# maffos/Diffusion-Modelling-for-inverse-problems

Hardware: NVIDIA B200
Metric: score-net evals/sec (posterior sampler) (higher is better)
Workload: dtype bf16

## Files before the change

### diffusion-modelling-for-inverse-problems_b200/csrc/dmip_rng.cuh

```cuda
#pragma once
#include <stdint.h>

namespace dmip {

constexpr uint32_t kPhiloxStepInit = 0xFFFFFFFFu;
constexpr uint32_t kStreamState = 0;
constexpr uint32_t kStreamObs = 1;

__device__ __forceinline__ void philox4x32_10(uint32_t c0, uint32_t c1, uint32_t c2, uint32_t c3, uint32_t k0,
                                              uint32_t k1, uint32_t (&out)[4]) {
#pragma unroll
  for (int r = 0; r < 10; ++r) {
    const uint32_t hi0 = __umulhi(0xD2511F53u, c0), lo0 = 0xD2511F53u * c0;
    const uint32_t hi1 = __umulhi(0xCD9E8D57u, c2), lo1 = 0xCD9E8D57u * c2;
    c0 = hi1 ^ c1 ^ k0;
    c1 = lo1;
    c2 = hi0 ^ c3 ^ k1;
    c3 = lo0;
    k0 += 0x9E3779B9u;
    k1 += 0xBB67AE85u;
  }
  out[0] = c0; out[1] = c1; out[2] = c2; out[3] = c3;
}

__device__ __forceinline__ float u01(uint32_t r) { return (static_cast<float>(r >> 8) + 0.5f) * (1.0f / 16777216.0f); }

__device__ __forceinline__ void philox_normal4(uint64_t gidx, uint32_t step, uint32_t stream, uint32_t quad,
                                               uint64_t seed, float (&z)[4]) {
  uint32_t r[4];
  philox4x32_10(static_cast<uint32_t>(gidx), static_cast<uint32_t>(gidx >> 32), step, (stream << 16) | quad,
                static_cast<uint32_t>(seed), static_cast<uint32_t>(seed >> 32), r);
#pragma unroll
  for (int j = 0; j < 2; ++j) {
    const float u1 = u01(r[2 * j]), u2 = u01(r[2 * j + 1]);
    float R;
    asm("sqrt.approx.ftz.f32 %0, %1;" : "=f"(R) : "f"(fmaxf(-2.0f * __logf(u1), 0.0f)));
    float s, c;
    __sincosf(6.283185307179586f * u2, &s, &c);
    z[2 * j] = R * c;
    z[2 * j + 1] = R * s;
  }
}

}
```

### diffusion-modelling-for-inverse-problems_b200/csrc/dmip_tc.cu

```cuda
#include <stdlib.h>

#include "dmip_common.h"
#include "dmip_ptx.cuh"
#include "dmip_rng.cuh"
#include "dmip_sde.cuh"

namespace dmip {

namespace {

constexpr int kTileM = 128;
constexpr int kStageBytes = 16384;
constexpr int kNumSlots = 6;
constexpr int kNumPairs = kNumSlots / 2;
constexpr int kPairBytes = 2 * kStageBytes;
constexpr int kHBytes = 131072;
constexpr int kThreads = 640;
constexpr int kRegsSmall = 32;
constexpr int kRegsRow = 112;
constexpr int kNumRowWarps = 16;
constexpr int kRowThreads = 512;
constexpr int kProducerWarp = 16;
constexpr int kMmaWarp = 17;
#ifndef DMIP_CLUSTER
#define DMIP_CLUSTER 2
#endif
constexpr int kCluster = DMIP_CLUSTER;
constexpr uint32_t kTmemCols = 512;
constexpr uint32_t kTmemH = 0;
constexpr uint32_t kTmemAcc = 256;
constexpr uint32_t kTmemL0 = kTmemH + 192;
#ifndef DMIP_L2_TAIL_TMEM
#define DMIP_L2_TAIL_TMEM 1
#endif
constexpr bool kL2TailTmem = DMIP_L2_TAIL_TMEM != 0;

constexpr int kOffH = 0;
constexpr int kOffB = kOffH + kHBytes;
constexpr int kOffB0 = kOffB + kNumSlots * kStageBytes;
constexpr int kOffB3 = kOffB0 + 2048;
constexpr int kOffBar = kOffB3 + 512;
constexpr int kNumBars = 2 * kNumPairs + 2 + 2 + 1 + 1 + 1 + 4 + 1;
constexpr int kOffTmem = kOffBar + kNumBars * 8;
constexpr int kSmemBytes = kOffTmem + 16;

enum { kModeSampler = 0, kModeForward = 1 };

struct TcNetDev {
  const uint8_t* stages;
  const float* b0;
  const float* b1;
  const float* b2;
  const float* b3;
  const float* w0c;
  int kb0, ksteps0, dv, split, l0_f16, outpad, n_const, n_stages;
  int l0_tmem;
};

struct TcParams {
  int mode, variant, n_nets;
  TcNetDev net[2];
  int xdim, ydim, n_obs, tiles_per_obs, S;
  long long n_per_obs, n_tiles;
  float T, bmin, bmax, mean, std, delta, sqrt_delta;
  int sde_kind, n_corr;
  float snr;
  const float* y;
  float* out;
  int rng_mode;
  unsigned long long seed, gidx_base;
  const float* x0;
  const float* noise;
  const float* ynoise;
  const float* fx;
  const float* fcond;
  const float* ft;
  int fx_dim, fcond_dim, out_dim;
  int dbg;
  int cluster;
  unsigned long long* tl;
  int tl_cap;
};

struct Bars {
  uint64_t* full;
  uint64_t* empty;
  uint64_t* acc_full;
  uint64_t* acc_empty;
  uint64_t* out_full;
  uint64_t* out_empty;
  uint64_t* sh_free;
  uint64_t* hready;
  uint64_t* a0_ready;
};

__device__ __forceinline__ int keep(int v) { return __shfl_sync(0xffffffffu, v, 0); }
__device__ __forceinline__ long long keep(long long v) {
  const unsigned lo = __shfl_sync(0xffffffffu, static_cast<unsigned>(v), 0);
  const unsigned hi = __shfl_sync(0xffffffffu, static_cast<unsigned>(static_cast<unsigned long long>(v) >> 32), 0);
  return static_cast<long long>((static_cast<unsigned long long>(hi) << 32) | lo);
}
template <class T>
__device__ __forceinline__ const T* keep(const T* p) {
  return reinterpret_cast<const T*>(keep(static_cast<long long>(reinterpret_cast<uintptr_t>(p))));
}

__device__ __forceinline__ uint32_t pin_here(uint32_t v) {
  asm volatile("" : "+r"(v) :: "memory");
  return v;
}

template <int kRegs>
__device__ __forceinline__ void reg_dealloc() { asm volatile("setmaxnreg.dec.sync.aligned.u32 %0;" ::"n"(kRegs)); }
template <int kRegs>
__device__ __forceinline__ void reg_alloc() { asm volatile("setmaxnreg.inc.sync.aligned.u32 %0;" ::"n"(kRegs)); }

__device__ __forceinline__ void st_shared_v4(void* p, uint32_t a, uint32_t b, uint32_t c, uint32_t d) {
  asm volatile("st.shared.v4.b32 [%0], {%1, %2, %3, %4};" ::"r"(smem_u32(p)), "r"(a), "r"(b), "r"(c), "r"(d) : "memory");
}

#ifndef DMIP_EPI
#define DMIP_EPI 1
#endif
template <bool kDoubleTanh>
__device__ __forceinline__ void tanh_pack16(const uint32_t (&v)[16], const float* __restrict__ bias, uint32_t (&pk)[8]) {
#pragma unroll
  for (int q = 0; q < 4; ++q) {
    const float4 bq = kDoubleTanh ? *reinterpret_cast<const float4*>(bias + q * 4)
                                  : __ldg(reinterpret_cast<const float4*>(bias + q * 4));
#ifndef DMIP_H_F16
    float a[4];
#pragma unroll
    for (int e = 0; e < 4; ++e) {
      const float bb = e == 0 ? bq.x : e == 1 ? bq.y : e == 2 ? bq.z : bq.w;
      float t = tanh_fast(__uint_as_float(v[q * 4 + e]) + bb);
      if (kDoubleTanh) t = tanh_unit_poly(t);
      a[e] = t;
    }
    pk[q * 2] = pack_bf16x2(a[0], a[1]);
    pk[q * 2 + 1] = pack_bf16x2(a[2], a[3]);
#else
#if DMIP_EPI == 0
    uint32_t t01 = tanh_f16x2(pack_f16x2(__uint_as_float(v[q * 4 + 0]) + bq.x, __uint_as_float(v[q * 4 + 1]) + bq.y));
    uint32_t t23 = tanh_f16x2(pack_f16x2(__uint_as_float(v[q * 4 + 2]) + bq.z, __uint_as_float(v[q * 4 + 3]) + bq.w));
    if (kDoubleTanh) {
      t01 = tanh_unit_poly_f16x2(t01);
      t23 = tanh_unit_poly_f16x2(t23);
    }
#elif DMIP_EPI == 1
    float a[4];
#pragma unroll
    for (int e = 0; e < 4; ++e) {
      const float bb = e == 0 ? bq.x : e == 1 ? bq.y : e == 2 ? bq.z : bq.w;
      float t = tanh_fast(__uint_as_float(v[q * 4 + e]) + bb);
      if (kDoubleTanh) t = tanh_unit_poly(t);
      a[e] = t;
    }
    uint32_t t01 = pack_f16x2(a[0], a[1]), t23 = pack_f16x2(a[2], a[3]);
#else
    float a[4];
#pragma unroll
    for (int e = 0; e < 4; ++e) {
      const float bb = e == 0 ? bq.x : e == 1 ? bq.y : e == 2 ? bq.z : bq.w;
      a[e] = tanh_fast(__uint_as_float(v[q * 4 + e]) + bb);
    }
    uint32_t t01 = pack_f16x2(a[0], a[1]), t23 = pack_f16x2(a[2], a[3]);
    if (kDoubleTanh) {
      t01 = tanh_unit_poly_f16x2(t01);
      t23 = tanh_unit_poly_f16x2(t23);
    }
#endif
    pk[q * 2] = t01;
    pk[q * 2 + 1] = t23;
#endif
  }
}

struct NoExtra {
  __device__ __forceinline__ void operator()() const {}
};

template <bool kDoubleTanh, bool kToTmem, class Extra = NoExtra>
__device__ __forceinline__ void epi_hidden(uint32_t lane_taddr, uint32_t acc_col, int cgp, int row, int chunk, int lane,
                                           const float* __restrict__ bias, uint8_t* sH, uint64_t* acc_empty,
                                           uint64_t* hready, Extra extra = NoExtra()) {
  const int n0 = chunk * 128 + cgp * 32;
  uint32_t v[16], pk[8];
  tmem_ld16(lane_taddr + acc_col + cgp * 32, v);
  tc_wait_ld();
  extra();
  tanh_pack16<kDoubleTanh>(v, bias + n0, pk);
  uint8_t* rowp = sH + (chunk * 2 + (cgp >> 1)) * kStageBytes + (row >> 3) * 1024 + (row & 7) * 128;
  const int c0 = (cgp & 1) * 4;
  if (kToTmem) {
    tmem_st8(lane_taddr + kTmemH + static_cast<uint32_t>(n0 >> 1), pk);
  } else {
    st_shared_v4(rowp + (((c0 + 0) ^ (row & 7)) << 4), pk[0], pk[1], pk[2], pk[3]);
    st_shared_v4(rowp + (((c0 + 1) ^ (row & 7)) << 4), pk[4], pk[5], pk[6], pk[7]);
  }
  tmem_ld16(lane_taddr + acc_col + cgp * 32 + 16, v);
  tc_wait_ld();
  tc_fence_before();
  __syncwarp();
  if (lane == 0) mbar_arrive(acc_empty);
  tanh_pack16<kDoubleTanh>(v, bias + n0 + 16, pk);
  if (kToTmem) {
    tmem_st8(lane_taddr + kTmemH + static_cast<uint32_t>(n0 >> 1) + 8, pk);
    tc_wait_st();
    tc_fence_before();
  } else {
    st_shared_v4(rowp + (((c0 + 2) ^ (row & 7)) << 4), pk[0], pk[1], pk[2], pk[3]);
    st_shared_v4(rowp + (((c0 + 3) ^ (row & 7)) << 4), pk[4], pk[5], pk[6], pk[7]);
    fence_proxy_async_smem();
  }
  __syncwarp();
  if (lane == 0) mbar_arrive(hready);
}

__device__ __forceinline__ void a0_store(uint8_t* sH, int row, int k, float v) {
  const uint32_t off = sw128_offset(static_cast<uint32_t>(row), static_cast<uint32_t>(k), kStageBytes);
  const unsigned short h = static_cast<unsigned short>(pack_bf16x2(v, 0.f) & 0xFFFFu);
  *reinterpret_cast<unsigned short*>(sH + off) = h;
}
__device__ __forceinline__ float f16_clamp(float v) { return fminf(fmaxf(v, -65504.f), 65504.f); }
__device__ __forceinline__ void a0_store_f16(uint8_t* sH, int row, int k, float v) {
  const uint32_t off = sw128_offset(static_cast<uint32_t>(row), static_cast<uint32_t>(k), kStageBytes);
  *reinterpret_cast<unsigned short*>(sH + off) = static_cast<unsigned short>(pack_f16x2(f16_clamp(v), 0.f) & 0xFFFFu);
}
__device__ __forceinline__ void a0_put(uint8_t* sH, int row, int idx, int dvp, int split, float v) {
  if (split == 4) { a0_store_f16(sH, row, idx, v); return; }
  const float hi = bf16_round(v);
  a0_store(sH, row, idx, hi);
  if (split >= 2) a0_store(sH, row, dvp + idx, v - hi);
  if (split >= 3) a0_store(sH, row, 2 * dvp + idx, hi);
}
__device__ __forceinline__ void a0_put8(uint8_t* sH, int row, int idx0, int dvp, int split, const float* v) {
  uint8_t* rowp0 = sH + (row >> 3) * 1024 + (row & 7) * 128;
  if (split == 4) {
    st_shared_v4(rowp0 + (idx0 >> 6) * kStageBytes + ((((idx0 & 63) >> 3) ^ (row & 7)) << 4),
                 pack_f16x2(f16_clamp(v[0]), f16_clamp(v[1])), pack_f16x2(f16_clamp(v[2]), f16_clamp(v[3])),
                 pack_f16x2(f16_clamp(v[4]), f16_clamp(v[5])), pack_f16x2(f16_clamp(v[6]), f16_clamp(v[7])));
    return;
  }
  float hi[8];
#pragma unroll
  for (int e = 0; e < 8; ++e) hi[e] = bf16_round(v[e]);
  const uint32_t h0 = pack_bf16x2(hi[0], hi[1]), h1 = pack_bf16x2(hi[2], hi[3]), h2 = pack_bf16x2(hi[4], hi[5]),
                 h3 = pack_bf16x2(hi[6], hi[7]);
  uint8_t* rowp = sH + (row >> 3) * 1024 + (row & 7) * 128;
  auto chunk_ptr = [&](int k) { return rowp + (k >> 6) * kStageBytes + ((((k & 63) >> 3) ^ (row & 7)) << 4); };
  st_shared_v4(chunk_ptr(idx0), h0, h1, h2, h3);
  if (split >= 2)
    st_shared_v4(chunk_ptr(dvp + idx0), pack_bf16x2(v[0] - hi[0], v[1] - hi[1]), pack_bf16x2(v[2] - hi[2], v[3] - hi[3]),
                 pack_bf16x2(v[4] - hi[4], v[5] - hi[5]), pack_bf16x2(v[6] - hi[6], v[7] - hi[7]));
  if (split >= 3) st_shared_v4(chunk_ptr(2 * dvp + idx0), h0, h1, h2, h3);
}

struct TlRole {
  unsigned long long* p;
  unsigned int n, cap;
  bool minimal;
};
__device__ __forceinline__ TlRole tl_role(const TcParams& P, int dbg, int role, bool on) {
  TlRole r;
  r.p = nullptr;
  r.n = 0;
  r.cap = 0;
  r.minimal = (dbg & 64) != 0;
  if (P.tl != nullptr && blockIdx.x == 0 && on) {
    const int seg = P.tl_cap / 4;
    r.p = P.tl + static_cast<size_t>(role) * seg;
    r.cap = static_cast<unsigned int>(seg - 1);
  }
  return r;
}
__device__ __forceinline__ void tl_mark_impl(TlRole& r, uint32_t code) {
  if (r.p != nullptr && r.n < r.cap && (!r.minimal || code == 0xD00u || (code & 0xF00u) == 0x100u || code == 0xE00u)) {
    r.p[1 + r.n] = (static_cast<unsigned long long>(clock64()) << 16) | code;
    ++r.n;
  }
}
__device__ __forceinline__ void tl_finish_impl(const TlRole& r) {
  if (r.p != nullptr) r.p[0] = r.n;
}
#ifdef DMIP_DEBUG
#define tl_mark(r, code) tl_mark_impl(r, code)
#define tl_finish(r) tl_finish_impl(r)
#define job_mark(r, code) ((void)0)
#elif defined(DMIP_JOBMARKS)
#define tl_mark(r, code) ((void)0)
#define tl_finish(r) tl_finish_impl(r)
#define job_mark(r, code) tl_mark_impl(r, code)
#else
#define tl_mark(r, code) ((void)0)
#define tl_finish(r) ((void)0)
#define job_mark(r, code) ((void)0)
#endif

template <int NP, int VAR>
__global__ void __launch_bounds__(kThreads, 1) k_tc_mlp(const __grid_constant__ TcParams P) {
  constexpr int kOwn = (NP + 3) / 4;
  constexpr bool cdiffe = (VAR == DMIP_CDIFFE);
  constexpr bool dps = (VAR == DMIP_DPS);
  extern __shared__ __align__(1024) uint8_t smem[];
  if ((smem_u32(smem) & 1023u) != 0u) __trap();
  uint8_t* sH = smem + kOffH;
  uint8_t* sB = smem + kOffB;
  float* sB0 = reinterpret_cast<float*>(smem + kOffB0);
  float* sB3 = reinterpret_cast<float*>(smem + kOffB3);
  uint64_t* bars = reinterpret_cast<uint64_t*>(smem + kOffBar);
  uint32_t* tmem_holder = reinterpret_cast<uint32_t*>(smem + kOffTmem);
  Bars B;
  B.full = bars;
  B.empty = bars + kNumPairs;
  B.acc_full = bars + 2 * kNumPairs;
  B.acc_empty = B.acc_full + 2;
  B.out_full = B.acc_empty + 2;
  B.out_empty = B.out_full + 1;
  B.sh_free = B.out_empty + 1;
  B.hready = B.sh_free + 1;
  B.a0_ready = B.hready + 4;

  const int warp = __shfl_sync(0xffffffffu, threadIdx.x >> 5, 0);
  const int lane = threadIdx.x & 31;

  if (warp == kProducerWarp && lane == 0) {
    for (int i = 0; i < kNumPairs; ++i) {
      mbar_init(&B.full[i], 1);
      mbar_init(&B.empty[i], static_cast<uint32_t>(kCluster));
    }
    for (int i = 0; i < 2; ++i) {
      mbar_init(&B.acc_full[i], 1);
      mbar_init(&B.acc_empty[i], kNumRowWarps);
    }
    mbar_init(B.out_full, 1);
    mbar_init(B.out_empty, kNumRowWarps);
    mbar_init(B.sh_free, 1);
    for (int i = 0; i < 4; ++i) mbar_init(&B.hready[i], kNumRowWarps);
    mbar_init(B.a0_ready, kNumRowWarps);
    fence_barrier_init();
  }
  if (warp == kMmaWarp) tmem_alloc<kTmemCols>(tmem_holder);
  for (int i = threadIdx.x; i < kHBytes / 16; i += kThreads) reinterpret_cast<uint4*>(sH)[i] = make_uint4(0, 0, 0, 0);
  for (int i = threadIdx.x; i < 128; i += kThreads) {
    if (dps) sB3[i] = i < 16 ? P.net[i >> 3].b3[i & 7] : 0.f;
    else sB3[i] = P.net[0].b3[i];
  }
  fence_proxy_async_smem();
  tc_fence_before();
  __syncthreads();
  tc_fence_after();
  const uint32_t tmem_base = __shfl_sync(0xffffffffu, *tmem_holder, 0);

  constexpr int C = kCluster;
#ifdef DMIP_DEBUG
  const int dbg = P.dbg & static_cast<int>(*reinterpret_cast<volatile uint32_t*>(tmem_holder) == 0xFFFFFFFFu ? 0u : 0xFFFFFFFFu);
#else
#ifndef DMIP_EXP
#define DMIP_EXP 0
#endif
  constexpr int dbg = DMIP_EXP;
#endif
  const int n_tiles = keep(static_cast<int>(P.n_tiles));
  const uint32_t crank = C > 1 ? cluster_ctarank() : 0u;
  const uint16_t cmask = static_cast<uint16_t>((1u << C) - 1u);
  if (C > 1) cluster_sync_all();
  const int tile_first = static_cast<int>(blockIdx.x / C) * C;
  const int tile_stride = keep(static_cast<int>(gridDim.x));

  const int n_pass = keep(P.n_nets);
  const int S = keep(P.S);
  const int n_steps = keep((P.mode == kModeSampler) ? S * (1 + P.n_corr) : 1);
  constexpr int n_ring = kNumPairs;

  if (warp >= kNumRowWarps) {
    reg_dealloc<kRegsSmall>();
    if (warp == kProducerWarp) {
      int s = 0;
      uint32_t ph = 0;
      TlRole tl = tl_role(P, dbg, 0, lane == 0);
      constexpr uint32_t part = kPairBytes / C;
      for (int tb = tile_first; tb < n_tiles; tb += tile_stride) {
        for (int step = 0; step < n_steps; ++step) {
          for (int p = 0; p < n_pass; ++p) {
            const uint8_t* src = keep(P.net[p].stages);
            const int npairs = keep(P.net[p].n_stages >> 1);
            for (int pr = 0; pr < npairs; ++pr) {
              mbar_wait(&B.empty[s], ph ^ 1u, 0x100 + s);
              tl_mark(tl, 0x600u | (pr & 0xFF));
              const uint8_t* g = src + static_cast<size_t>(pr) * kPairBytes;
              if (elect_one()) {
                if (dbg & 1) {
                  mbar_arrive(&B.full[s]);
                } else {
                  mbar_arrive_expect_tx(&B.full[s], kPairBytes);
                  if (C == 1)
                    bulk_g2s(sB + s * kPairBytes, g, kPairBytes, &B.full[s]);
                  else
                    bulk_g2s_multicast(sB + s * kPairBytes + crank * part, g + crank * part, part, &B.full[s], cmask);
                }
              }
              __syncwarp();
              if (++s == n_ring) { s = 0; ph ^= 1u; }
            }
          }
        }
      }
      tl_finish(tl);
    } else if (warp == kMmaWarp) {
      int s = 0;
      uint32_t ph = 0;
      uint32_t job = 0;
      uint32_t hr_par = 0;
      uint32_t a0_par = 0;
      uint32_t ch0 = 0, ch1 = 0, n_out = 0;
      uint32_t lastkind = 0;
      uint32_t blk = 0;
      TlRole tl = tl_role(P, dbg, 1, lane == 0);
      const uint32_t a_base = (smem_u32(sH) & 0x3FFFFu) >> 4;
      const uint32_t b_base = (smem_u32(sB) & 0x3FFFFu) >> 4;
      const uint64_t desc_hi = umma_smem_desc_sw128(0) & 0xFFFFFFFF00000000ull;
      constexpr uint32_t kBlk16 = kStageBytes >> 4, kPair16 = kPairBytes >> 4;

      auto acquire_acc = [&](int buf, bool is_out, int jl) {
        const uint32_t lk = (lastkind >> (2 * buf)) & 3u;
        tl_mark(tl, 0xB00u | jl);
        if (lk == 1u) mbar_wait(&B.acc_empty[buf], ((buf ? ch1 : ch0) - 1u) & 1u, 0x300 + buf);
        else if (lk == 2u) mbar_wait(B.out_empty, (n_out - 1u) & 1u, 0x310 + buf);
        tl_mark(tl, 0x100u | jl);
        job_mark(tl, 0x100u | jl);
        if (is_out) ++n_out; else { if (buf) ++ch1; else ++ch0; }
        lastkind = (lastkind & ~(3u << (2 * buf))) | ((is_out ? 2u : 1u) << (2 * buf));
      };

      for (int tb = tile_first; tb < n_tiles; tb += tile_stride) {
        for (int step = 0; step < n_steps; ++step) {
          for (int p = 0; p < n_pass; ++p) {
            const int net_kb0 = keep(P.net[p].kb0), net_ksteps0 = keep(P.net[p].ksteps0);
            const uint32_t idesc_out = umma_idesc_bf16(128, static_cast<uint32_t>(keep(P.net[p].outpad)));
            constexpr uint32_t idesc_hid = umma_idesc_bf16(128, 128);
            const uint32_t idesc_l0 = keep(P.net[p].l0_f16) ? umma_idesc_f16(128, 128) : idesc_hid;
            const bool net_l0_tmem = keep(P.net[p].l0_tmem) != 0;
            tl_mark(tl, 0xD00u);
            job_mark(tl, 0xD00u);
            mbar_wait(B.a0_ready, a0_par, 0x200);
            tl_mark(tl, 0xE00u);
            a0_par ^= 1u;
            int jl = 0;
            blk = 0;
#pragma unroll 1
            for (int c = 0; c < 4; ++c, ++job, ++jl) {
              const int buf = job & 1;
              acquire_acc(buf, false, jl);
              const uint32_t d_tmem = tmem_base + kTmemAcc + buf * 128;
#pragma unroll 1
              for (int kb = 0; kb < net_kb0; ++kb, ++blk) {
                const uint32_t half = blk & 1u;
                if (half == 0u) mbar_wait(&B.full[s], ph, 0x500 + s);
                tc_fence_after();
                const int nk = (kb == net_kb0 - 1) ? (net_ksteps0 - 4 * (net_kb0 - 1)) : 4;
                const uint32_t b_lo = b_base + s * kPair16 + half * kBlk16;
                const uint32_t a_lo = a_base + kb * kBlk16;
                if (elect_one()) {
                  if (!(dbg & 2)) {
                    if (net_l0_tmem) {
                      const uint32_t a_tm = tmem_base + kTmemL0 + kb * 32;
#pragma unroll
                      for (int kk = 0; kk < 4; ++kk)
                        if (kk < nk) umma_ts(d_tmem, a_tm + kk * 8, desc_hi | (b_lo + kk * 2), idesc_l0, (kb | kk) != 0 ? 1u : 0u);
                    } else {
#pragma unroll
                      for (int kk = 0; kk < 4; ++kk)
                        if (kk < nk)
                          umma_ss(d_tmem, desc_hi | (a_lo + kk * 2), desc_hi | (b_lo + kk * 2), idesc_l0, (kb | kk) != 0 ? 1u : 0u);
                    }
                  }
                  if (half == 1u) tc_commit_multicast(&B.empty[s], cmask);
                  if (kb == net_kb0 - 1) tc_commit(&B.acc_full[buf]);
                }
                __syncwarp();
                if (half == 1u) { if (++s == n_ring) { s = 0; ph ^= 1u; } }
              }
              tl_mark(tl, 0x200u | jl);
              job_mark(tl, 0x200u | jl);
            }
#pragma unroll 1
            for (int l = 1; l < 4; ++l) {
              const int n_chunks = (l == 3) ? 1 : 4;
#ifndef DMIP_H_F16
              const uint32_t idesc = (l == 3) ? idesc_out : idesc_hid;
#else
              const uint32_t idesc = ((l == 3) ? idesc_out : idesc_hid) & ~((7u << 7) | (7u << 10));
#endif
#pragma unroll 1
              for (int c = 0; c < n_chunks; ++c, ++job, ++jl) {
                const int buf = job & 1;
                acquire_acc(buf, l == 3, jl);
                const uint32_t d_tmem = tmem_base + kTmemAcc + buf * 128;
#pragma unroll 1
                for (int pr = 0; pr < 4; ++pr) {
                  if (c == 0) {
                    mbar_wait(&B.hready[pr], (hr_par >> pr) & 1u, 0x400 + pr);
                    hr_par ^= 1u << pr;
                  }
                  mbar_wait(&B.full[s], ph, 0x500 + s);
                  tc_fence_after();
                  const uint32_t b_lo = b_base + s * kPair16;
                  if (elect_one()) {
                    if (!(dbg & 2)) {
                      if (l == 2 && !(kL2TailTmem && pr == 3)) {
                        const uint32_t a_lo = a_base + pr * kPair16;
#pragma unroll
                        for (int j = 0; j < 8; ++j)
                          umma_ss(d_tmem, desc_hi | (a_lo + (j >> 2) * kBlk16 + (j & 3) * 2),
                                  desc_hi | (b_lo + (j >> 2) * kBlk16 + (j & 3) * 2), idesc, (pr | j) != 0 ? 1u : 0u);
                      } else {
                        const uint32_t a_tm = tmem_base + kTmemH + pr * 64;
#pragma unroll
                        for (int j = 0; j < 8; ++j)
                          umma_ts(d_tmem, a_tm + j * 8, desc_hi | (b_lo + (j >> 2) * kBlk16 + (j & 3) * 2), idesc,
                                  (pr | j) != 0 ? 1u : 0u);
                      }
                    }
                    tc_commit_multicast(&B.empty[s], cmask);
                    if (pr == 3) {
                      if (l == 3) tc_commit(B.out_full);
                      else tc_commit(&B.acc_full[buf]);
                      if (l == 2 && c == 3) tc_commit(B.sh_free);
                    }
                  }
                  __syncwarp();
                  if (++s == n_ring) { s = 0; ph ^= 1u; }
                }
                tl_mark(tl, 0x200u | jl);
                job_mark(tl, 0x200u | jl);
              }
            }
          }
        }
      }
      tl_finish(tl);
    }
  } else {
    reg_alloc<kRegsRow>();
    const int quarter = warp & 3;
    const int cgp = warp >> 2;
    const int row = quarter * 32 + lane;
    const int et = threadIdx.x;
    const uint32_t lane_taddr = tmem_base + (static_cast<uint32_t>(quarter * 32) << 16);
    if (P.net[0].l0_tmem && cgp == 0) {
      const uint32_t z[16] = {0, 0, 0, 0, 0, 0, 0, 0, 0, 0, 0, 0, 0, 0, 0, 0};
#pragma unroll
      for (int c0 = 0; c0 < 64; c0 += 16) tmem_st16(lane_taddr + kTmemL0 + c0, z);
      tc_wait_st();
    }
    asm volatile("bar.sync 2, 512;" ::: "memory");
    TlRole tl = tl_role(P, dbg, warp == 0 ? 2 : 3, lane == 0 && (warp == 0 || warp == 12));
    uint32_t job = 0;
    uint32_t npass = 0;
    uint32_t cf0 = 0, cf1 = 0;
    const SdeSched sch = {P.sde_kind, S, P.n_corr, P.T, P.bmin, P.bmax, P.snr, P.delta, P.sqrt_delta};
    const TcNetDev& net_last = P.net[n_pass - 1];
    const int dvp = (net_last.dv + 7) & ~7;
    const int split = P.net[0].l0_f16 ? 4 : P.net[0].split;
    const bool l0_tmem = P.net[0].l0_tmem != 0;
    const bool sampler = (P.mode == kModeSampler);
    const int xdim = P.xdim;
    const int np = sampler ? (xdim + 7) >> 3 : 0;
    const int pbase = np >> 2, prem = np & 3;
    const int n_own = pbase + (cgp < prem ? 1 : 0);
    const int piece_lo = cgp * pbase + (cgp < prem ? cgp : prem);
    float xs[kOwn * 8];
    float yt[cdiffe ? 8 : 1];
    float myU[2], myWt[2];
#pragma unroll
    for (int j = 0; j < kOwn * 8; ++j) xs[j] = 0.f;
#pragma unroll
    for (int j = 0; j < (cdiffe ? 8 : 1); ++j) yt[j] = 0.f;
    myU[0] = myU[1] = myWt[0] = myWt[1] = 0.f;

    for (int tb = tile_first; tb < n_tiles; tb += tile_stride) {
      const bool tile_ok = tb + static_cast<int>(crank) < n_tiles;
      const int tile = tile_ok ? tb + static_cast<int>(crank) : n_tiles - 1;
      const int obs = static_cast<int>(tile / P.tiles_per_obs);
      const long long prow = static_cast<long long>(tile % P.tiles_per_obs) * kTileM + row;
      const bool valid = tile_ok && prow < P.n_per_obs;
      const long long grow = static_cast<long long>(obs) * P.n_per_obs + prow;
      const unsigned long long gidx = P.gidx_base + static_cast<unsigned long long>(grow);

      auto diffuse_y = [&](int stp) {
        if (!cdiffe) return;
        float g2u, alpha, var;
        sde_terms<true>(sch, sde_substep_tau(sch, stp), g2u, alpha, var);
        const float sd = sqrtf(var);
#pragma unroll
        for (int h = 0; h < 2; ++h) {
          const int q = cgp + 4 * h;
          if (q * 4 < P.ydim) {
            float z[4] = {0.f, 0.f, 0.f, 0.f};
            if (P.rng_mode == DMIP_RNG_PHILOX) philox_normal4(gidx, pin_here(static_cast<uint32_t>(stp)), kStreamObs, q, P.seed, z);
#pragma unroll
            for (int e = 0; e < 4; ++e) {
              const int jj = q * 4 + e;
              float v = 0.f;
              if (valid && jj < P.ydim) {
                const float eta = P.rng_mode == DMIP_RNG_PHILOX
                                      ? z[e]
                                      : P.ynoise[(static_cast<long long>(stp) * (static_cast<long long>(P.n_obs) * P.n_per_obs) + grow) * P.ydim + jj];
                v = fmaf(sd, eta, alpha * P.y[obs * P.ydim + jj]);
              }
              yt[cdiffe ? h * 4 + e : 0] = v;
            }
          }
        }
      };
      auto put_yt = [&]() {
        if (!cdiffe) return;
#pragma unroll
        for (int h = 0; h < 2; ++h)
#pragma unroll
          for (int e = 0; e < 4; ++e) {
            const int jj = (cgp + 4 * h) * 4 + e;
            if (jj < P.ydim) a0_put(sH, row, xdim + jj, dvp, split, yt[cdiffe ? h * 4 + e : 0]);
          }
      };
      auto put_x = [&]() {
#pragma unroll
        for (int i = 0; i < kOwn; ++i) {
          if (i < n_own) {
            const int pc = piece_lo + i;
            if (l0_tmem) {
              const float* v = &xs[i * 8];
              tmem_st4(lane_taddr + kTmemL0 + static_cast<uint32_t>(pc * 4),
                       pack_f16x2(f16_clamp(v[0]), f16_clamp(v[1])), pack_f16x2(f16_clamp(v[2]), f16_clamp(v[3])),
                       pack_f16x2(f16_clamp(v[4]), f16_clamp(v[5])), pack_f16x2(f16_clamp(v[6]), f16_clamp(v[7])));
            } else if (cdiffe) {
#pragma unroll
              for (int e = 0; e < 8; ++e)
                if (pc * 8 + e < xdim) a0_put(sH, row, pc * 8 + e, dvp, split, xs[i * 8 + e]);
            } else {
              a0_put8(sH, row, pc * 8, dvp, split, &xs[i * 8]);
            }
          }
        }
      };

      auto publish_a0 = [&]() {
        if (l0_tmem) {
          tc_wait_st();
          tc_fence_before();
        } else {
          fence_proxy_async_smem();
        }
        __syncwarp();
        if (lane == 0) mbar_arrive(B.a0_ready);
      };

      if (sampler) {
        for (int p = 0; p < n_pass; ++p) {
          const TcNetDev& net = P.net[p];
          float u = net.b0[et];
          const float* wr = net.w0c + static_cast<size_t>(et) * net.n_const;
          for (int j = 0; j + 1 < net.n_const; ++j) u = fmaf(wr[j], P.y[obs * P.ydim + j], u);
          const float wt = wr[net.n_const - 1];
          if (p == 0) { myU[0] = u; myWt[0] = wt; } else if (dps) { myU[1] = u; myWt[1] = wt; }
          if (p == 0) sB0[et] = fmaf(sde_substep_tau(sch, 0), wt, u);
        }
#pragma unroll
        for (int i = 0; i < kOwn; ++i) {
          if (i < n_own) {
            const int pc = piece_lo + i;
#pragma unroll
            for (int h = 0; h < 2; ++h) {
              float z4[4] = {0.f, 0.f, 0.f, 0.f};
              if (P.rng_mode == DMIP_RNG_PHILOX) philox_normal4(gidx, kPhiloxStepInit, kStreamState, pc * 2 + h, P.seed, z4);
#pragma unroll
              for (int e = 0; e < 4; ++e) {
                const int j = pc * 8 + h * 4 + e;
                float v = 0.f;
                if (valid && j < xdim) {
                  const float zz = P.rng_mode == DMIP_RNG_PHILOX ? z4[e] : P.x0[grow * xdim + j];
                  v = zz * P.std + P.mean;
                }
                xs[i * 8 + h * 4 + e] = v;
              }
            }
          }
        }
        put_x();
        if (cdiffe) {
          diffuse_y(0);
          put_yt();
        }
      } else {
        const TcNetDev& net = P.net[0];
        sB0[et] = net.b0[et];
        if (valid) {
          for (int k = cgp; k < net.dv; k += 4) {
            float v;
            if (k < P.fx_dim) v = P.fx[grow * P.fx_dim + k];
            else if (k < P.fx_dim + P.fcond_dim) v = P.fcond[grow * P.fcond_dim + (k - P.fx_dim)];
            else v = P.ft[grow];
            a0_put(sH, row, k, dvp, split, v);
          }
        }
      }
      publish_a0();
      tl_mark(tl, 0x500u);

      for (int step = 0; step < n_steps; ++step) {
        const SdeCoef co = sde_coef<true>(sch, step, dps);
        const float tau = co.tau;
        const bool last_step = (step == n_steps - 1);
        float stash[dps ? 8 : 1];
#pragma unroll
        for (int e = 0; e < (dps ? 8 : 1); ++e) stash[e] = 0.f;

        for (int p = 0; p < n_pass; ++p, ++npass) {
          const TcNetDev& net = P.net[p];
          const bool last_pass = (p == n_pass - 1);
          const bool fuse_draw = sampler && last_pass && !(dbg & 16) && P.rng_mode == DMIP_RNG_PHILOX;
          float zdraw[4] = {0.f, 0.f, 0.f, 0.f}, zdraw4[4] = {0.f, 0.f, 0.f, 0.f};
          int jl = 0;
#pragma unroll 1
          for (int l = 0; l < 3; ++l) {
            const float* bias = (l == 0) ? sB0 : (l == 1 ? net.b1 : net.b2);
#pragma unroll 1
            for (int c = 0; c < 4; ++c, ++job, ++jl) {
              const int buf = job & 1;
              job_mark(tl, 0x600u | jl);
              mbar_wait(&B.acc_full[buf], (buf ? cf1 : cf0) & 1u, 0x800 + buf);
              if (buf) ++cf1; else ++cf0;
              tc_fence_after();
              tl_mark(tl, 0x300u | jl);
              job_mark(tl, 0x300u | jl);
              const uint32_t acc_col = kTmemAcc + buf * 128;
              if (dbg & 8) {
                tc_fence_before();
                __syncwarp();
                if (lane == 0) { mbar_arrive(&B.acc_empty[buf]); mbar_arrive(&B.hready[c]); }
              } else if (l == 0)
                epi_hidden<true, true>(lane_taddr, acc_col, cgp, row, c, lane, bias, sH, &B.acc_empty[buf], &B.hready[c]);
              else {
                const int ip = (l - 1) * 2 + (c >> 1);
                const bool draw_here = fuse_draw && (c & 1) == 0 && ip < kOwn;
                const int pc = piece_lo + ip;
                auto draw = [&]() {
                  const uint32_t here = pin_here(static_cast<uint32_t>(step));
                  philox_normal4(gidx, here, kStreamState, pc * 2, P.seed, zdraw);
                  philox_normal4(gidx, here, kStreamState, pc * 2 + 1, P.seed, zdraw4);
                };
                if (l == 1 && !(kL2TailTmem && c == 3)) {
                  if (draw_here)
                    epi_hidden<false, false>(lane_taddr, acc_col, cgp, row, c, lane, bias, sH, &B.acc_empty[buf], &B.hready[c], draw);
                  else
                    epi_hidden<false, false>(lane_taddr, acc_col, cgp, row, c, lane, bias, sH, &B.acc_empty[buf], &B.hready[c]);
                } else {
                  if (draw_here)
                    epi_hidden<false, true>(lane_taddr, acc_col, cgp, row, c, lane, bias, sH, &B.acc_empty[buf], &B.hready[c], draw);
                  else
                    epi_hidden<false, true>(lane_taddr, acc_col, cgp, row, c, lane, bias, sH, &B.acc_empty[buf], &B.hready[c]);
                }
              }
              tl_mark(tl, 0x400u | jl);
              job_mark(tl, 0x400u | jl);
              if (sampler && last_pass && !(dbg & 16)) {
                if (l >= 1 && (c & 1) == 0) {
#pragma unroll
                  for (int i = 0; i < kOwn; ++i) {
                    if (i == (l - 1) * 2 + (c >> 1) && i < n_own) {
                      const int pc = piece_lo + i;
                      const float ca = co.ca;
                      const float* b3s = sB3 + (dps ? 8 : pc * 8);
                      const float4 q0 = *reinterpret_cast<const float4*>(b3s);
                      const float4 q1 = *reinterpret_cast<const float4*>(b3s + 4);
                      const float b3v[8] = {q0.x, q0.y, q0.z, q0.w, q1.x, q1.y, q1.z, q1.w};
                      float za[4], zb[4];
#pragma unroll
                      for (int e = 0; e < 4; ++e) { za[e] = zdraw[e]; zb[e] = zdraw4[e]; }
                      const float kx = co.kx, ke = co.ke;
#pragma unroll
                      for (int e = 0; e < 8; ++e) {
                        const int j = pc * 8 + e;
                        float eps = 0.f;
                        if (valid && j < xdim)
                          eps = fuse_draw ? (e < 4 ? za[e & 3] : zb[e & 3])
                                          : P.noise[(static_cast<long long>(step) * (static_cast<long long>(P.n_obs) * P.n_per_obs) + grow) * xdim + j];
                        const float xv = xs[i * 8 + e];
                        xs[i * 8 + e] = fmaf(kx, xv, xv) + fmaf(ke, eps, ca * b3v[e]);
                      }
                    }
                  }
                }
                if (l == 2 && c == 1 && cdiffe && !last_step) diffuse_y(step + 1);
              }
            }
          }
          tl_mark(tl, 0x310u);
          mbar_wait(B.sh_free, npass & 1u, 0x600);
          if (sampler) {
            const bool wrap = (p + 1 == n_pass);
            const float tau_n = wrap ? sde_substep_tau(sch, step + 1) : tau;
            const float u = (wrap || !dps) ? myU[0] : myU[1];
            const float wt = (wrap || !dps) ? myWt[0] : myWt[1];
            sB0[et] = fmaf(tau_n, wt, u);
          }
          if (sampler) {
            if (!last_pass && !l0_tmem) {
              put_x();
              publish_a0();
            } else if (cdiffe && !last_step) {
              put_yt();
            }
          }
          tl_mark(tl, 0x320u);
          mbar_wait(B.out_full, npass & 1u, 0x700);
          tc_fence_after();
          tl_mark(tl, 0x300u | 12);
          job_mark(tl, 0x300u | 12);
          const uint32_t acc_col = kTmemAcc + (job & 1u) * 128;
          ++job;
          if (!sampler) {
            const float* b3 = net.b3;
            for (int pc = cgp; pc * 8 < P.out_dim; pc += 4) {
              uint32_t v[8];
              tmem_ld8(lane_taddr + acc_col + pc * 8, v);
              tc_wait_ld();
#pragma unroll
              for (int e = 0; e < 8; ++e) {
                const int j = pc * 8 + e;
                if (valid && j < P.out_dim) P.out[grow * P.out_dim + j] = __uint_as_float(v[e]) + b3[j];
              }
            }
          } else if (!last_pass) {
            if (n_own > 0) {
              uint32_t v[8];
              tmem_ld8(lane_taddr + acc_col, v);
              tc_wait_ld();
#pragma unroll
              for (int e = 0; e < 8; ++e) stash[dps ? e : 0] = __uint_as_float(v[e]) + sB3[e];
            }
            if (l0_tmem) {
              put_x();
              publish_a0();
            }
          } else {
            const float ca = co.ca;
            uint32_t v[kOwn][8];
#pragma unroll
            for (int i = 0; i < kOwn; ++i)
              if (i < n_own) tmem_ld8(lane_taddr + acc_col + (piece_lo + i) * 8, v[i]);
            tc_wait_ld();
#pragma unroll
            for (int i = 0; i < kOwn; ++i) {
              if (i < n_own) {
#pragma unroll
                for (int e = 0; e < 8; ++e) {
                  float a = __uint_as_float(v[i][e]);
                  if (dps) a += stash[dps ? e : 0];
                  xs[i * 8 + e] = fmaf(ca, a, xs[i * 8 + e]);
                }
              }
            }
          }
          tc_fence_before();
          __syncwarp();
          if (lane == 0) mbar_arrive(B.out_empty);
          tl_mark(tl, 0x400u | 12);
          job_mark(tl, 0x400u | 12);
          if (sampler && last_pass) {
            if (last_step) {
              if (valid) {
#pragma unroll
                for (int i = 0; i < kOwn; ++i)
                  if (i < n_own) {
#pragma unroll
                    for (int e = 0; e < 8; ++e) {
                      const int j = (piece_lo + i) * 8 + e;
                      if (j < xdim) P.out[grow * xdim + j] = xs[i * 8 + e];
                    }
                  }
              }
            } else {
              put_x();
              publish_a0();
              tl_mark(tl, 0x500u);
              job_mark(tl, 0x500u);
            }
          }
        }
      }
    }
    tl_finish(tl);
  }

  tc_fence_before();
  __syncthreads();
  if (C > 1) cluster_sync_all();
  if (warp == kMmaWarp) {
    tc_fence_after();
    tmem_dealloc<kTmemCols>(tmem_base);
  }
}

int fill_net(const DmipMlp* net, const void* packed, int n_varying, int out_rows, int split, TcNetDev* o) {
  TcNetGeom g;
  int rc = tc_net_geom(net, n_varying, out_rows, split, &g);
  if (rc) return rc;
  const uint8_t* base = static_cast<const uint8_t*>(packed);
  const float* tail = reinterpret_cast<const float*>(base + g.stage_bytes());
  o->stages = base;
  o->b0 = tail;
  o->b1 = tail + 512;
  o->b2 = tail + 1024;
  o->b3 = tail + 1536;
  o->w0c = tail + 1664;
  o->kb0 = g.kb0;
  o->ksteps0 = g.k0pad / 16;
  o->dv = g.n_varying;
  o->split = g.split;
  o->l0_f16 = g.l0_f16;
  o->l0_tmem = 0;
  o->outpad = g.outpad;
  o->n_const = g.n_const;
  o->n_stages = g.n_stages;
  return 0;
}

int g_n_sm = 0;
int g_dbg = 0;
unsigned long long* g_tl = nullptr;
int g_tl_cap = 0;

bool g_dev_ready[64] = {};

int init_device() {
  int dev = 0;
  DMIP_CHECK_CUDA(cudaGetDevice(&dev));
  if (dev < 0 || dev >= 64 || !g_dev_ready[dev]) {
    DMIP_CHECK_CUDA(cudaDeviceGetAttribute(&g_n_sm, cudaDevAttrMultiProcessorCount, dev));
#define DMIP_SET_SMEM(NP, VAR) \
  DMIP_CHECK_CUDA(cudaFuncSetAttribute(k_tc_mlp<NP, VAR>, cudaFuncAttributeMaxDynamicSharedMemorySize, kSmemBytes))
    DMIP_SET_SMEM(1, DMIP_CDE);
    DMIP_SET_SMEM(1, DMIP_CDIFFE);
    DMIP_SET_SMEM(1, DMIP_DPS);
    DMIP_SET_SMEM(4, DMIP_CDE);
    DMIP_SET_SMEM(4, DMIP_CDIFFE);
    DMIP_SET_SMEM(13, DMIP_CDE);
#undef DMIP_SET_SMEM
    if (getenv("DMIP_DBG")) g_dbg = atoi(getenv("DMIP_DBG"));
    if (dev >= 0 && dev < 64) g_dev_ready[dev] = true;
  }
  return DMIP_OK;
}

int launch(TcParams& P, cudaStream_t s) {
  int rc = init_device();
  if (rc) return rc;
  const int n_sm = g_n_sm;
  P.tl = g_tl;
  P.tl_cap = g_tl_cap;
  if (P.n_tiles <= 0) return DMIP_OK;
  DMIP_REQUIRE(P.n_tiles < (1LL << 31), "too many particle tiles in one call (%lld); split the call", P.n_tiles);
  const int C = kCluster;
  P.cluster = C;
  P.dbg = g_dbg;
  const long long want_clusters = (P.n_tiles + C - 1) / C;
  const long long max_clusters = n_sm / C;
  const long long n_clusters = want_clusters < max_clusters ? want_clusters : max_clusters;
  cudaLaunchConfig_t cfg = {};
  cfg.gridDim = dim3(static_cast<unsigned>(n_clusters * C));
  cfg.blockDim = dim3(kThreads);
  cfg.dynamicSmemBytes = kSmemBytes;
  cfg.stream = s;
  cudaLaunchAttribute attr[1];
  attr[0].id = cudaLaunchAttributeClusterDimension;
  attr[0].val.clusterDim.x = static_cast<unsigned>(C);
  attr[0].val.clusterDim.y = 1;
  attr[0].val.clusterDim.z = 1;
  cfg.attrs = attr;
  cfg.numAttrs = 1;
  const int state_cols = (P.mode == kModeSampler) ? P.xdim : 1;
  const int var = (P.mode == kModeSampler) ? P.variant : DMIP_CDE;
  if (var == DMIP_DPS) {
    DMIP_CHECK_CUDA(cudaLaunchKernelEx(&cfg, k_tc_mlp<1, DMIP_DPS>, P));
  } else if (var == DMIP_CDIFFE) {
    if (state_cols <= 8) DMIP_CHECK_CUDA(cudaLaunchKernelEx(&cfg, k_tc_mlp<1, DMIP_CDIFFE>, P));
    else DMIP_CHECK_CUDA(cudaLaunchKernelEx(&cfg, k_tc_mlp<4, DMIP_CDIFFE>, P));
  } else {
    if (state_cols <= 8) DMIP_CHECK_CUDA(cudaLaunchKernelEx(&cfg, k_tc_mlp<1, DMIP_CDE>, P));
    else if (state_cols <= 32) DMIP_CHECK_CUDA(cudaLaunchKernelEx(&cfg, k_tc_mlp<4, DMIP_CDE>, P));
    else DMIP_CHECK_CUDA(cudaLaunchKernelEx(&cfg, k_tc_mlp<13, DMIP_CDE>, P));
  }
  DMIP_CHECK_CUDA(cudaGetLastError());
  count_launch();
  return DMIP_OK;
}

}

size_t sampler_tc_workspace() {
  return 256;
}

void tcl_debug_set_timeline(unsigned long long* buf, int cap);
void debug_set_timeline(unsigned long long* buf, int cap) {
  g_tl = buf;
  g_tl_cap = cap;
  tcl_debug_set_timeline(buf, cap);
}

int launch_sampler_tc(const DmipSampler* d, cudaStream_t s) {
  TcParams P = {};
  DMIP_REQUIRE(d->xdim <= 104, "tcgen05 sampler keeps the state in registers: xdim <= 104 (got %d); use DMIP_PREC_F32", d->xdim);
  if (d->variant == DMIP_CDIFFE)
    DMIP_REQUIRE(d->xdim <= 32 && d->ydim <= 24, "tcgen05 CDiffE sampler supports xdim <= 32, ydim <= 24 (got %d, %d); "
                 "use DMIP_PREC_F32", d->xdim, d->ydim);
  P.mode = kModeSampler;
  P.variant = d->variant;
  const int dv = d->variant == DMIP_CDIFFE ? d->xdim + d->ydim : d->xdim;
  int rc;
  if (d->variant == DMIP_DPS) {
    P.n_nets = 2;
    DMIP_REQUIRE(d->packed2 != nullptr, "DPS sampler needs packed2 (prior_net image)");
    DMIP_REQUIRE(d->xdim <= 8, "DPS tcgen05 sampler supports xdim <= 8 (got %d)", d->xdim);
    if ((rc = fill_net(&d->net2, d->packed2, d->xdim, d->xdim, d->l0_split, &P.net[0]))) return rc;
    if ((rc = fill_net(&d->net, d->packed, d->xdim, d->xdim, d->l0_split, &P.net[1]))) return rc;
  } else {
    P.n_nets = 1;
    if ((rc = fill_net(&d->net, d->packed, dv, d->xdim, d->l0_split, &P.net[0]))) return rc;
  }
  for (int p = 0; p < P.n_nets; ++p)
    P.net[p].l0_tmem = (P.net[p].l0_f16 && d->variant != DMIP_CDIFFE && P.net[p].ksteps0 * 16 <= 128) ? 1 : 0;
  P.xdim = d->xdim;
  P.ydim = d->ydim;
  P.n_obs = d->n_obs;
  P.n_per_obs = d->n_per_obs;
  P.tiles_per_obs = static_cast<int>((d->n_per_obs + kTileM - 1) / kTileM);
  P.n_tiles = static_cast<long long>(P.tiles_per_obs) * d->n_obs;
  P.S = d->num_steps;
  P.T = d->T;
  P.sde_kind = d->sde_kind;
  P.bmin = d->sde_kind == DMIP_SDE_VE ? d->sigma_min : d->beta_min;
  P.bmax = d->sde_kind == DMIP_SDE_VE ? d->sigma_max : d->beta_max;
  P.n_corr = d->n_corrector;
  P.snr = d->snr;
  P.mean = d->mean;
  P.std = d->std;
  const double delta = static_cast<double>(d->T) / d->num_steps;
  P.delta = static_cast<float>(delta);
  P.sqrt_delta = static_cast<float>(sqrt(delta));
  P.y = d->y;
  P.out = d->out;
  P.rng_mode = d->rng_mode;
  P.seed = d->seed;
  P.gidx_base = d->gidx_base;
  P.x0 = d->x0;
  P.noise = d->noise;
  P.ynoise = d->ynoise;
  return launch(P, s);
}

int launch_forward_tc(const DmipForward* d, cudaStream_t s) {
  TcParams P = {};
  P.mode = kModeForward;
  P.variant = DMIP_CDE;
  P.n_nets = 1;
  int rc;
  if ((rc = fill_net(&d->net, d->packed, d->net.in_dim, d->net.out_dim, d->l0_split, &P.net[0]))) return rc;
  P.n_obs = 1;
  P.n_per_obs = d->n;
  P.tiles_per_obs = static_cast<int>((d->n + kTileM - 1) / kTileM);
  P.n_tiles = P.tiles_per_obs;
  P.S = 1;
  P.T = 1.f;
  P.out = d->out;
  P.fx = d->x;
  P.fcond = d->cond;
  P.ft = d->t;
  P.fx_dim = d->x_dim;
  P.fcond_dim = d->cond_dim;
  P.out_dim = d->net.out_dim;
  return launch(P, s);
}

}
```

Before: 819.4 million.

## Offload Philox noise generation to dedicated warps with smem double buffer

Adds dedicated noise-producer warps (warps 18+) that generate Gaussian noise with Philox into a double-buffered shared-memory region. The row warps then read it through new mbarrier full/empty/gate handshakes instead of drawing it inline in the epilogue. It also precomputes the first two Philox rounds per row and step as a prefix, so each draw only runs the remaining rounds. The aim is to take RNG and Box-Muller arithmetic off the critical epilogue path. In exchange it adds barrier synchronisation, reuses part of the H smem region (block 6 onward), and disables itself when layer-0 weights would overlap that region.

```diff
diff --git a/diffusion-modelling-for-inverse-problems_b200/csrc/dmip_rng.cuh b/diffusion-modelling-for-inverse-problems_b200/csrc/dmip_rng.cuh
--- a/diffusion-modelling-for-inverse-problems_b200/csrc/dmip_rng.cuh
+++ b/diffusion-modelling-for-inverse-problems_b200/csrc/dmip_rng.cuh
@@ -7,29 +7,35 @@
 constexpr uint32_t kStreamState = 0;
 constexpr uint32_t kStreamObs = 1;
 
+constexpr uint32_t kPhiloxM0 = 0xD2511F53u, kPhiloxM1 = 0xCD9E8D57u;
+constexpr uint32_t kPhiloxW0 = 0x9E3779B9u, kPhiloxW1 = 0xBB67AE85u;
+
+template <int kFirst>
+__device__ __forceinline__ void philox_rounds(uint32_t (&c)[4], uint32_t k0, uint32_t k1) {
+  k0 += kFirst * kPhiloxW0;
+  k1 += kFirst * kPhiloxW1;
+#pragma unroll
+  for (int r = kFirst; r < 10; ++r) {
+    const uint32_t hi0 = __umulhi(kPhiloxM0, c[0]), lo0 = kPhiloxM0 * c[0];
+    const uint32_t hi1 = __umulhi(kPhiloxM1, c[2]), lo1 = kPhiloxM1 * c[2];
+    c[0] = hi1 ^ c[1] ^ k0;
+    c[1] = lo1;
+    c[2] = hi0 ^ c[3] ^ k1;
+    c[3] = lo0;
+    k0 += kPhiloxW0;
+    k1 += kPhiloxW1;
+  }
+}
+
 __device__ __forceinline__ void philox4x32_10(uint32_t c0, uint32_t c1, uint32_t c2, uint32_t c3, uint32_t k0,
                                               uint32_t k1, uint32_t (&out)[4]) {
-#pragma unroll
-  for (int r = 0; r < 10; ++r) {
-    const uint32_t hi0 = __umulhi(0xD2511F53u, c0), lo0 = 0xD2511F53u * c0;
-    const uint32_t hi1 = __umulhi(0xCD9E8D57u, c2), lo1 = 0xCD9E8D57u * c2;
-    c0 = hi1 ^ c1 ^ k0;
-    c1 = lo1;
-    c2 = hi0 ^ c3 ^ k1;
-    c3 = lo0;
-    k0 += 0x9E3779B9u;
-    k1 += 0xBB67AE85u;
-  }
   out[0] = c0; out[1] = c1; out[2] = c2; out[3] = c3;
+  philox_rounds<0>(out, k0, k1);
 }
 
 __device__ __forceinline__ float u01(uint32_t r) { return (static_cast<float>(r >> 8) + 0.5f) * (1.0f / 16777216.0f); }
 
-__device__ __forceinline__ void philox_normal4(uint64_t gidx, uint32_t step, uint32_t stream, uint32_t quad,
-                                               uint64_t seed, float (&z)[4]) {
-  uint32_t r[4];
-  philox4x32_10(static_cast<uint32_t>(gidx), static_cast<uint32_t>(gidx >> 32), step, (stream << 16) | quad,
-                static_cast<uint32_t>(seed), static_cast<uint32_t>(seed >> 32), r);
+__device__ __forceinline__ void box_muller4(const uint32_t (&r)[4], float (&z)[4]) {
 #pragma unroll
   for (int j = 0; j < 2; ++j) {
     const float u1 = u01(r[2 * j]), u2 = u01(r[2 * j + 1]);
@@ -42,4 +48,36 @@
   }
 }
 
+__device__ __forceinline__ void philox_normal4(uint64_t gidx, uint32_t step, uint32_t stream, uint32_t quad,
+                                               uint64_t seed, float (&z)[4]) {
+  uint32_t r[4];
+  philox4x32_10(static_cast<uint32_t>(gidx), static_cast<uint32_t>(gidx >> 32), step, (stream << 16) | quad,
+                static_cast<uint32_t>(seed), static_cast<uint32_t>(seed >> 32), r);
+  box_muller4(r, z);
 }
+
+struct PhiloxPrefix {
+  uint32_t c2x;
+  uint32_t c1k;
+  uint32_t c2, c3;
+};
+__device__ __forceinline__ PhiloxPrefix philox_prefix(uint32_t pa_hi, uint32_t pa_lo, uint32_t gidx_hi, uint32_t st_hi,
+                                                      uint32_t st_lo, uint64_t seed) {
+  const uint32_t k0 = static_cast<uint32_t>(seed), k1 = static_cast<uint32_t>(seed >> 32);
+  const uint32_t a0 = st_hi ^ gidx_hi ^ k0;
+  PhiloxPrefix q;
+  q.c2x = pa_hi ^ k1;
+  q.c1k = st_lo ^ (k0 + kPhiloxW0);
+  q.c2 = __umulhi(kPhiloxM0, a0) ^ pa_lo ^ (k1 + kPhiloxW1);
+  q.c3 = kPhiloxM0 * a0;
+  return q;
+}
+__device__ __forceinline__ void philox_normal4_pre(const PhiloxPrefix& q, uint32_t stream, uint32_t quad, uint64_t seed,
+                                                   float (&z)[4]) {
+  const uint32_t a2 = q.c2x ^ ((stream << 16) | quad);
+  uint32_t c[4] = {__umulhi(kPhiloxM1, a2) ^ q.c1k, kPhiloxM1 * a2, q.c2, q.c3};
+  philox_rounds<2>(c, static_cast<uint32_t>(seed), static_cast<uint32_t>(seed >> 32));
+  box_muller4(c, z);
+}
+
+}
diff --git a/diffusion-modelling-for-inverse-problems_b200/csrc/dmip_tc.cu b/diffusion-modelling-for-inverse-problems_b200/csrc/dmip_tc.cu
--- a/diffusion-modelling-for-inverse-problems_b200/csrc/dmip_tc.cu
+++ b/diffusion-modelling-for-inverse-problems_b200/csrc/dmip_tc.cu
@@ -22,6 +22,7 @@
 constexpr int kRowThreads = 512;
 constexpr int kProducerWarp = 16;
 constexpr int kMmaWarp = 17;
+constexpr int kNoiseWarp0 = 18;
 #ifndef DMIP_CLUSTER
 #define DMIP_CLUSTER 2
 #endif
@@ -34,13 +35,20 @@
 #define DMIP_L2_TAIL_TMEM 1
 #endif
 constexpr bool kL2TailTmem = DMIP_L2_TAIL_TMEM != 0;
+#ifndef DMIP_NOISE_WARPS
+#define DMIP_NOISE_WARPS 1
+#endif
+constexpr bool kNoiseWarps = DMIP_NOISE_WARPS != 0;
+constexpr int kNoiseBlock0 = 6;
+constexpr int kDbgEpilogueDraw = 128;
+__host__ __device__ constexpr bool noise_from_warps(int ip, int own) { return own == 1 || ip == 3; }
 
 constexpr int kOffH = 0;
 constexpr int kOffB = kOffH + kHBytes;
 constexpr int kOffB0 = kOffB + kNumSlots * kStageBytes;
 constexpr int kOffB3 = kOffB0 + 2048;
 constexpr int kOffBar = kOffB3 + 512;
-constexpr int kNumBars = 2 * kNumPairs + 2 + 2 + 1 + 1 + 1 + 4 + 1;
+constexpr int kNumBars = 2 * kNumPairs + 2 + 2 + 1 + 1 + 1 + 4 + 1 + 2 + 2 + 1;
 constexpr int kOffTmem = kOffBar + kNumBars * 8;
 constexpr int kSmemBytes = kOffTmem + 16;
 
@@ -68,6 +76,7 @@
   const float* y;
   float* out;
   int rng_mode;
+  int noise_warps;
   unsigned long long seed, gidx_base;
   const float* x0;
   const float* noise;
@@ -92,7 +101,26 @@
   uint64_t* sh_free;
   uint64_t* hready;
   uint64_t* a0_ready;
+  uint64_t* noise_full;
+  uint64_t* noise_empty;
+  uint64_t* noise_gate;
 };
+
+struct TileRow {
+  int obs;
+  long long grow;
+  bool valid;
+};
+__device__ __forceinline__ TileRow tile_row(const TcParams& P, int tb, uint32_t crank, int n_tiles, int row) {
+  const bool tile_ok = tb + static_cast<int>(crank) < n_tiles;
+  const int tile = tile_ok ? tb + static_cast<int>(crank) : n_tiles - 1;
+  TileRow r;
+  r.obs = static_cast<int>(tile / P.tiles_per_obs);
+  const long long prow = static_cast<long long>(tile % P.tiles_per_obs) * kTileM + row;
+  r.valid = tile_ok && prow < P.n_per_obs;
+  r.grow = static_cast<long long>(r.obs) * P.n_per_obs + prow;
+  return r;
+}
 
 __device__ __forceinline__ int keep(int v) { return __shfl_sync(0xffffffffu, v, 0); }
 __device__ __forceinline__ long long keep(long long v) {
@@ -320,6 +348,9 @@
   B.sh_free = B.out_empty + 1;
   B.hready = B.sh_free + 1;
   B.a0_ready = B.hready + 4;
+  B.noise_full = B.a0_ready + 1;
+  B.noise_empty = B.noise_full + 2;
+  B.noise_gate = B.noise_empty + 2;
 
   const int warp = __shfl_sync(0xffffffffu, threadIdx.x >> 5, 0);
   const int lane = threadIdx.x & 31;
@@ -338,6 +369,11 @@
     mbar_init(B.sh_free, 1);
     for (int i = 0; i < 4; ++i) mbar_init(&B.hready[i], kNumRowWarps);
     mbar_init(B.a0_ready, kNumRowWarps);
+    for (int i = 0; i < 2; ++i) {
+      mbar_init(&B.noise_full[i], 2);
+      mbar_init(&B.noise_empty[i], kNumRowWarps);
+    }
+    mbar_init(B.noise_gate, kNumRowWarps);
     fence_barrier_init();
   }
   if (warp == kMmaWarp) tmem_alloc<kTmemCols>(tmem_holder);
@@ -372,6 +408,8 @@
   const int S = keep(P.S);
   const int n_steps = keep((P.mode == kModeSampler) ? S * (1 + P.n_corr) : 1);
   constexpr int n_ring = kNumPairs;
+  const bool gen_noise = kNoiseWarps && P.noise_warps != 0 && !(dbg & 16);
+  uint8_t* sNoise = sH + kNoiseBlock0 * kStageBytes;
 
   if (warp >= kNumRowWarps) {
     reg_dealloc<kRegsSmall>();
@@ -540,6 +578,54 @@
         }
       }
       tl_finish(tl);
+    } else if (gen_noise) {
+      const int gt = (warp - kNoiseWarp0) * 32 + lane;
+      const unsigned long long seed = P.seed;
+      const int np = (P.xdim + 7) >> 3;
+      const int pbase = np >> 2, prem = np & 3;
+      uint32_t g = 0;
+      for (int tb = tile_first; tb < n_tiles; tb += tile_stride) {
+        unsigned long long gidx[2];
+#pragma unroll
+        for (int j = 0; j < 2; ++j)
+          gidx[j] = P.gidx_base + static_cast<unsigned long long>(tile_row(P, tb, crank, n_tiles, gt + 64 * j).grow);
+#pragma unroll 1
+        for (int step = 0; step < n_steps; ++step) {
+          const uint32_t st_hi = __umulhi(kPhiloxM1, static_cast<uint32_t>(step));
+          const uint32_t st_lo = kPhiloxM1 * static_cast<uint32_t>(step);
+#pragma unroll 1
+          for (int ip = 0; ip < kOwn; ++ip) {
+            if (!noise_from_warps(ip, kOwn)) continue;
+            if (kOwn > 1) mbar_wait(B.noise_gate, g & 1u, 0x910);
+            const uint32_t slot = g & 1u;
+            mbar_wait(&B.noise_empty[slot], ((g >> 1) & 1u) ^ 1u, 0x900 + slot);
+            float4* dst = reinterpret_cast<float4*>(sNoise + slot * kStageBytes);
+            auto draw_row = [&](unsigned long long gi, int r) {
+              const uint32_t glo = static_cast<uint32_t>(gi);
+              const PhiloxPrefix pre_r = philox_prefix(__umulhi(kPhiloxM0, glo), kPhiloxM0 * glo,
+                                                       static_cast<uint32_t>(gi >> 32), st_hi, st_lo, seed);
+#pragma unroll 1
+              for (int cg = 0; cg < 4; ++cg) {
+                const int n_own = pbase + (cg < prem ? 1 : 0);
+                if (ip < n_own) {
+                  const int pc = cg * pbase + (cg < prem ? cg : prem) + ip;
+#pragma unroll
+                  for (int h = 0; h < 2; ++h) {
+                    float z[4];
+                    philox_normal4_pre(pre_r, kStreamState, static_cast<uint32_t>(pc * 2 + h), seed, z);
+                    dst[(cg * 2 + h) * kTileM + r] = make_float4(z[0], z[1], z[2], z[3]);
+                  }
+                }
+              }
+            };
+            draw_row(gidx[0], gt);
+            draw_row(gidx[1], gt + 64);
+            __syncwarp();
+            if (lane == 0) mbar_arrive(&B.noise_full[slot]);
+            ++g;
+          }
+        }
+      }
     }
   } else {
     reg_alloc<kRegsRow>();
@@ -580,12 +666,10 @@
     myU[0] = myU[1] = myWt[0] = myWt[1] = 0.f;
 
     for (int tb = tile_first; tb < n_tiles; tb += tile_stride) {
-      const bool tile_ok = tb + static_cast<int>(crank) < n_tiles;
-      const int tile = tile_ok ? tb + static_cast<int>(crank) : n_tiles - 1;
-      const int obs = static_cast<int>(tile / P.tiles_per_obs);
-      const long long prow = static_cast<long long>(tile % P.tiles_per_obs) * kTileM + row;
-      const bool valid = tile_ok && prow < P.n_per_obs;
-      const long long grow = static_cast<long long>(obs) * P.n_per_obs + prow;
+      const TileRow tr = tile_row(P, tb, crank, n_tiles, row);
+      const int obs = tr.obs;
+      const bool valid = tr.valid;
+      const long long grow = tr.grow;
       const unsigned long long gidx = P.gidx_base + static_cast<unsigned long long>(grow);
 
       auto diffuse_y = [&](int stp) {
@@ -743,7 +827,7 @@
                 epi_hidden<true, true>(lane_taddr, acc_col, cgp, row, c, lane, bias, sH, &B.acc_empty[buf], &B.hready[c]);
               else {
                 const int ip = (l - 1) * 2 + (c >> 1);
-                const bool draw_here = fuse_draw && (c & 1) == 0 && ip < kOwn;
+                const bool draw_here = fuse_draw && (c & 1) == 0 && ip < kOwn && !(gen_noise && noise_from_warps(ip, kOwn));
                 const int pc = piece_lo + ip;
                 auto draw = [&]() {
                   const uint32_t here = pin_here(static_cast<uint32_t>(step));
@@ -764,7 +848,23 @@
               }
               tl_mark(tl, 0x400u | jl);
               job_mark(tl, 0x400u | jl);
+              if (gen_noise && kOwn > 1 && last_pass && l == 1 && c == 3) {
+                __syncwarp();
+                if (lane == 0) mbar_arrive(B.noise_gate);
+              }
               if (sampler && last_pass && !(dbg & 16)) {
+                const int ip = (l - 1) * 2 + (c >> 1);
+                if (gen_noise && l >= 1 && (c & 1) == 0 && ip < kOwn && noise_from_warps(ip, kOwn)) {
+                  const uint32_t gn = dps ? npass >> 1 : npass;
+                  const uint32_t slot = gn & 1u;
+                  mbar_wait(&B.noise_full[slot], (gn >> 1) & 1u, 0x820 + slot);
+                  const float4* src = reinterpret_cast<const float4*>(sNoise + slot * kStageBytes);
+                  const float4 n0 = src[(cgp * 2) * kTileM + row], n1 = src[(cgp * 2 + 1) * kTileM + row];
+                  __syncwarp();
+                  if (lane == 0) mbar_arrive(&B.noise_empty[slot]);
+                  zdraw[0] = n0.x; zdraw[1] = n0.y; zdraw[2] = n0.z; zdraw[3] = n0.w;
+                  zdraw4[0] = n1.x; zdraw4[1] = n1.y; zdraw4[2] = n1.z; zdraw4[3] = n1.w;
+                }
                 if (l >= 1 && (c & 1) == 0) {
 #pragma unroll
                   for (int i = 0; i < kOwn; ++i) {
@@ -928,7 +1028,6 @@
 }
 
 int g_n_sm = 0;
-int g_dbg = 0;
 unsigned long long* g_tl = nullptr;
 int g_tl_cap = 0;
 
@@ -948,7 +1047,6 @@
     DMIP_SET_SMEM(4, DMIP_CDIFFE);
     DMIP_SET_SMEM(13, DMIP_CDE);
 #undef DMIP_SET_SMEM
-    if (getenv("DMIP_DBG")) g_dbg = atoi(getenv("DMIP_DBG"));
     if (dev >= 0 && dev < 64) g_dev_ready[dev] = true;
   }
   return DMIP_OK;
@@ -964,7 +1062,9 @@
   DMIP_REQUIRE(P.n_tiles < (1LL << 31), "too many particle tiles in one call (%lld); split the call", P.n_tiles);
   const int C = kCluster;
   P.cluster = C;
-  P.dbg = g_dbg;
+  const char* dbg_env = getenv("DMIP_DBG");
+  P.dbg = dbg_env ? atoi(dbg_env) : 0;
+  if (P.dbg & kDbgEpilogueDraw) P.noise_warps = 0;
   const long long want_clusters = (P.n_tiles + C - 1) / C;
   const long long max_clusters = n_sm / C;
   const long long n_clusters = want_clusters < max_clusters ? want_clusters : max_clusters;
@@ -1032,6 +1132,9 @@
   }
   for (int p = 0; p < P.n_nets; ++p)
     P.net[p].l0_tmem = (P.net[p].l0_f16 && d->variant != DMIP_CDIFFE && P.net[p].ksteps0 * 16 <= 128) ? 1 : 0;
+  P.noise_warps = (kNoiseWarps && kL2TailTmem && d->rng_mode == DMIP_RNG_PHILOX) ? 1 : 0;
+  for (int p = 0; p < P.n_nets; ++p)
+    if (!P.net[p].l0_tmem && P.net[p].kb0 > kNoiseBlock0) P.noise_warps = 0;
   P.xdim = d->xdim;
   P.ydim = d->ydim;
   P.n_obs = d->n_obs;
```

Result: no change. 816.9 million (median of 6 runs) (-0.3%).
